# pdpatel13/Gravity-Simulator-using-MPI-Spark-and-CUDA

Measured on AMD Instinct MI355X. Metric: body-updates/sec (whole node) at N=1M direct O(N^2), 1/2/4/8 MI355X, higher is better.
Workload: dtype fp32

## Files before the change

### csrc/hip/nbody_sym.hip

```cpp
#include <hip/hip_runtime.h>
#include <stdint.h>
#include <stdlib.h>

#include "gravsim.h"
#include "gs_common.h"
#include "gs_kernels.h"
#include "gs_sym_tile.h"

namespace gs {
namespace {

template <typename T>
struct Shape;
template <>
struct Shape<float> {
  static constexpr int I = 8, W = kSymC / (64 * I), J = 2;
};
template <>
struct Shape<double> {
  static constexpr int W = 4, I = 8, J = 1;
};

template <typename T>
struct Geo {
  static constexpr int W = Shape<T>::W, I = Shape<T>::I, J = Shape<T>::J;
  static constexpr int kTileI = 64 * I;
  static constexpr int kTileJ = 64 * J;
  static constexpr int kThreads = 64 * W;
  static constexpr int kTilesPerChunk = kSymC / kTileJ;
  static constexpr int kTilesPerQuantum = 128 / kTileJ;
  static_assert(W * kTileI == kSymC, "one workgroup holds one chunk on its i side");
  static_assert(kTileJ <= 128 && 128 % kTileJ == 0, "a j-tile must not straddle quanta");
};

__device__ __forceinline__ int shell_len(int A, int NC) {
  const bool takes = (A < NC / 2) == ((A & 1) == 0);
  return takes ? NC / 2 : NC / 2 - 1;
}

template <typename T>
struct TileSeq {
  int A, NC, real_chunks, u, u1;
  bool diag;
  static constexpr int kT = Geo<T>::kTilesPerChunk;
  __device__ __forceinline__ int d() const { return diag ? 0 : 1 + u / kT; }
  __device__ __forceinline__ int t() const { return u % kT; }
  __device__ __forceinline__ int valid(int uu) const {
    if (!diag)
      while (uu < u1 && (A + 1 + uu / kT) % NC >= real_chunks) uu = (uu / kT + 1) * kT;
    return uu;
  }
  __device__ __forceinline__ bool done() const { return u >= u1; }
  __device__ __forceinline__ int64_t row0() const {
    const int B = diag ? A : (A + d()) % NC;
    return (int64_t)B * kSymC + t() * Geo<T>::kTileJ;
  }
  __device__ __forceinline__ void next() { u = valid(u + 1); }
};

template <typename V>
__device__ __forceinline__ void stage_store(V* dst, int b, const V& q) {
  const int j = b / 64, l = b % 64;
  dst[j * sym::kStagedRows + sym::staged_entry(l, 0)] = q;
  dst[j * sym::kStagedRows + sym::staged_entry(l, 1)] = q;
}

template <typename T>
constexpr bool kJpack = sizeof(T) == 4;

template <typename T>
using ISetK = typename std::conditional<kJpack<T>, sym::ISetP<Geo<T>::I>,
                                        sym::ISetT<T, Geo<T>::I>>::type;

template <typename T>
struct StageQ {
  static constexpr int kN = kJpack<T> ? 2 : 1;
  static constexpr int kThreads = kJpack<T> ? 64 : Geo<T>::kTileJ;
  sym::Vec4<T> q[kN];
  __device__ __forceinline__ void load(const sym::Vec4<T>* X4, int64_t row0, int t) {
#pragma unroll
    for (int k = 0; k < kN; ++k) q[k] = X4[row0 + k * 64 + t];
  }
  __device__ __forceinline__ void store(sym::Vec4<T>* dst, int t) const {
    if constexpr (kJpack<T>) {
      const float4 p0 = {q[0].x, q[1].x, q[0].y, q[1].y}, p1 = {q[0].z, q[1].z, q[0].w, q[1].w};
#pragma unroll
      for (int c = 0; c < 2; ++c) {
        const int e = sym::staged_entry(t, c);
        dst[2 * e] = p0;
        dst[2 * e + 1] = p1;
      }
    } else {
      stage_store(dst, t, q[0]);
    }
  }
};

template <typename T>
struct Smem {
  T slot[2][Geo<T>::W][3][Geo<T>::kTileJ];
  sym::Vec4<T> jt[2][Geo<T>::J * sym::kStagedRows];
};

template <typename T, bool SYM, bool EXACT>
__device__ __forceinline__ void run_tiles(const SymArgs& a, ISetK<T>& is, TileSeq<T> seq,
                                          int br, Smem<T>& sm) {
  using G = Geo<T>;
  using V4 = sym::Vec4<T>;
  constexpr int J = G::J;
  const int w = threadIdx.x >> 6, lane = threadIdx.x & 63;
  const V4* X4 = static_cast<const V4*>(a.X);
  const T eps2 = (T)a.eps2, cut2 = (T)a.cut2;
  int buf = 0, cur = 0;
  const bool stager = threadIdx.x < StageQ<T>::kThreads;
  if (!seq.done() && stager) {
    StageQ<T> sq;
    sq.load(X4, seq.row0(), threadIdx.x);
    sq.store(sm.jt[0], threadIdx.x);
  }
  __syncthreads();
  while (!seq.done()) {
    TileSeq<T> nx = seq;
    nx.next();
    const int d = seq.d(), t = seq.t();
    StageQ<T> q_next;
    const bool stage_next = !nx.done() && stager;
    if (stage_next) q_next.load(X4, nx.row0(), threadIdx.x);
    T cx[J], cy[J], cz[J];
    sym::CSetT<T, J> cs;
#pragma unroll
    for (int j = 0; j < J; ++j) cs.cx[j] = cs.cy[j] = cs.cz[j] = T(0);
    if constexpr (kJpack<T>) {
      sym::tile_lds_jp<G::I, SYM, EXACT>(is, cs, sm.jt[cur], eps2, sym::f2{a.cut_k, a.cut_c});
    } else {
      sym::tile_lds64<G::I, SYM, EXACT>(is, cs, sm.jt[cur], eps2, cut2);
    }
#pragma unroll
    for (int j = 0; j < J; ++j) { cx[j] = cs.cx[j]; cy[j] = cs.cy[j]; cz[j] = cs.cz[j]; }
    if constexpr (SYM) {
#pragma unroll
      for (int j = 0; j < J; ++j) {
        sm.slot[buf][w][0][j * 64 + lane] = cx[j];
        sm.slot[buf][w][1][j * 64 + lane] = cy[j];
        sm.slot[buf][w][2][j * 64 + lane] = cz[j];
      }
    }
    if (stage_next) q_next.store(sm.jt[cur ^ 1], threadIdx.x);
    __syncthreads();
    if constexpr (SYM) {
      T* pj = static_cast<T*>(a.Pj) + ((int64_t)br * a.H + (d - 1)) * 3 * kSymC;
      for (int v = threadIdx.x; v < 3 * G::kTileJ; v += G::kThreads) {
        const int c = v / G::kTileJ, b = v % G::kTileJ;
        T acc = sm.slot[buf][0][c][b];
#pragma unroll
        for (int u = 1; u < G::W; ++u) acc += sm.slot[buf][u][c][b];
        pj[(int64_t)c * kSymC + t * G::kTileJ + b] = acc;
      }
      buf ^= 1;
    }
    cur ^= 1;
    seq = nx;
  }
}

__device__ __forceinline__ bool local_first_unit(const SymArgs& a, int b, int* br, int* s,
                                                 int* stage, int* part) {
  const uint32_t m = (uint32_t)a.lf[b];
  const bool ring = a.gate_n > 1, halves = a.Kr > 0 && !ring;
  *br = (int)((m >> kUnitRowShift) & (uint32_t)kUnitRowMax);
  *s = (int)(m & (uint32_t)kUnitMax);
  *stage = ring ? (int)((m >> 28) & 7u) : 0;
  *part = halves && ((m >> 30) & 1u) ? (int)((m >> 28) & 3u) : -1;
  return (m >> 31) != 0u;
}

__device__ __forceinline__ bool gate_open_or_defer(const SymArgs& a, int b, int stage) {
  __shared__ int open_s;
  if (threadIdx.x == 0) {
    const bool open =
        __hip_atomic_load(a.gate + stage, __ATOMIC_ACQUIRE, __HIP_MEMORY_SCOPE_SYSTEM) != 0u;
    if (!open) {
      const unsigned k =
          __hip_atomic_fetch_add(a.defer, 1u, __ATOMIC_RELAXED, __HIP_MEMORY_SCOPE_AGENT);
      a.defer[1 + k] = (unsigned)b;
    }
    open_s = open ? 1 : 0;
  }
  __syncthreads();
  return open_s != 0;
}

__device__ __forceinline__ void audit_unit(const SymArgs& a, unsigned long long n = 1) {
  if (threadIdx.x == 0)
    __hip_atomic_fetch_add(a.audit, n, __ATOMIC_RELAXED, __HIP_MEMORY_SCOPE_AGENT);
}

template <typename T, bool EXACT>
__device__ __forceinline__ unsigned force_sym_body(const SymArgs& a, int b) {
  using G = Geo<T>;
  using V4 = sym::Vec4<T>;
  __shared__ Smem<T> sm;
  const int w = threadIdx.x >> 6, lane = threadIdx.x & 63;
  int br, s, stage = 0, part = -1;
  bool gated = false;
  if (a.units == 6) {
    gated = local_first_unit(a, b, &br, &s, &stage, &part) && a.gate != nullptr;
  } else if (a.units == 7) {
    local_first_unit(a, (int)a.defer[1 + a.defer_index], &br, &s, &stage, &part);
  } else {
    const int ns = a.S - a.Kr, shell = a.band_rows * ns, dg = a.band_rows * a.D;
    if (b < shell) {
      br = b / ns;
      s = b % ns;
    } else if (b < shell + dg) {
      const int k = b - shell;
      br = k / a.D;
      s = a.S + k % a.D;
    } else {
      const int k = b - shell - dg;
      part = k % a.Np;
      br = (k / a.Np) / a.Kr;
      s = ns + (k / a.Np) % a.Kr;
    }
  }
  const int A = a.a0 + a.band0 + br;
  const bool diag = s >= a.S;
  const bool split = !diag && s >= a.S - a.Kr;
  const unsigned long long weight = split && part < 0 ? (unsigned long long)a.Np : 1ull;
  const bool count_empty = a.audit != nullptr;
  if ((int64_t)A * kSymC >= a.n_real)
    return count_empty ? (unsigned)weight : 0u;
  const int seg_tiles = a.L * G::kTilesPerQuantum;
  TileSeq<T> seq{A, a.NC, a.real_chunks, 0, 0, diag};
  int u_lo = 0;
  if (diag) {
    const int q = s - a.S, plen = G::kTilesPerChunk / a.D;
    seq.u = q * plen;
    seq.u1 = seq.u + plen;
  } else {
    const int h_tiles = shell_len(A, a.NC) * G::kTilesPerChunk;
    const int u0 = s * seg_tiles;
    if (u0 >= h_tiles)
      return count_empty ? (unsigned)weight : 0u;
    seq.u1 = min(u0 + seg_tiles, h_tiles);
    u_lo = u0;
    seq.u = seq.valid(u0);
  }
  if (gated && !gate_open_or_defer(a, b, stage)) return 0u;
  const unsigned long long t_start = a.utrace ? __builtin_amdgcn_s_memrealtime() : 0ull;
  const V4* X4 = static_cast<const V4*>(a.X);
  ISetK<T> is;
  const int64_t i_row0 = (int64_t)A * kSymC + w * G::kTileI;
#pragma unroll
  for (int i = 0; i < G::I; ++i) {
    const V4 q = X4[i_row0 + i * 64 + lane];
    is.x[i] = q.x; is.y[i] = q.y; is.z[i] = q.z; is.mu[i] = q.w;
    is.ax[i] = is.ay[i] = is.az[i] = std::remove_reference_t<decltype(is.ax[i])>(0);
  }
  auto store_i = [&](T* out) {
#pragma unroll
    for (int i = 0; i < G::I; ++i) {
      const int b = w * G::kTileI + i * 64 + lane;
      if constexpr (kJpack<T>) {
        out[b] = is.ax[i].x + is.ax[i].y;
        out[kSymC + b] = is.ay[i].x + is.ay[i].y;
        out[2 * kSymC + b] = is.az[i].x + is.az[i].y;
      } else {
        out[b] = is.ax[i];
        out[kSymC + b] = is.ay[i];
        out[2 * kSymC + b] = is.az[i];
      }
    }
  };
  if (diag) {
    run_tiles<T, false, EXACT>(a, is, seq, br, sm);
    store_i(static_cast<T*>(a.Pd) + ((int64_t)br * a.D + (s - a.S)) * 3 * kSymC);
  } else {
    T* const pi = static_cast<T*>(a.Pi) + ((int64_t)br * a.S + s) * 3 * kSymC;
    T* const px = split ? static_cast<T*>(a.Px) +
                              ((int64_t)br * a.Kr + (s - (a.S - a.Kr))) * (a.Np - 1) * 3 * kSymC
                        : nullptr;
    const int pc0 = split && part > 0 ? part : 0;
    const int pc1 = !split ? 1 : part >= 0 ? part + 1 : a.Np;
    const int u_end = seq.u1;
#pragma unroll 1
    for (int pc = pc0; pc < pc1; ++pc) {
      TileSeq<T> sq = seq;
      if (split) {
        sq.u1 = min(u_lo + (pc + 1) * seg_tiles / a.Np, u_end);
        sq.u = sq.valid(min(u_lo + pc * seg_tiles / a.Np, u_end));
      }
      if (pc > pc0) {
#pragma unroll
        for (int i = 0; i < G::I; ++i)
          is.ax[i] = is.ay[i] = is.az[i] = std::remove_reference_t<decltype(is.ax[i])>(0);
      }
      run_tiles<T, true, EXACT>(a, is, sq, br, sm);
      store_i(pc == 0 ? pi : px + (int64_t)(pc - 1) * 3 * kSymC);
      if (pc + 1 < pc1) __syncthreads();

    }
  }
  if (a.utrace && threadIdx.x == 0) {
    const unsigned hw = __builtin_amdgcn_s_getreg((31 << 11) | 4);
    const unsigned xcc = __builtin_amdgcn_s_getreg((3 << 11) | 20);
    const int64_t slot = a.units == 7 ? (int64_t)a.trace_defer0 + a.defer_index : b;
    unsigned long long* e = a.utrace + 4 * slot;
    e[0] = t_start;
    e[1] = __builtin_amdgcn_s_memrealtime();
    e[2] = (unsigned long long)hw | ((unsigned long long)xcc << 32);
    e[3] = ((unsigned long long)(unsigned)br << 32) | (unsigned)s;
  }
  return a.audit ? (unsigned)weight : 0u;
}

struct ClockSpan {
  __device__ __forceinline__ static unsigned long long* slot() {
    __shared__ unsigned long long t0[3];
    return t0;
  }
  __device__ __forceinline__ static void begin(const SymArgs& a) {
    if (threadIdx.x == 0) {
      slot()[2] = reinterpret_cast<unsigned long long>(a.clk);
      if (a.clk) {
        slot()[0] = __builtin_amdgcn_s_memtime();
        slot()[1] = __builtin_amdgcn_s_memrealtime();
      }
    }
  }
  __device__ __forceinline__ static void end() {
    if (threadIdx.x == 0) {
      unsigned long long* clk = reinterpret_cast<unsigned long long*>(slot()[2]);
      if (clk) {
        const unsigned long long mt1 = __builtin_amdgcn_s_memtime();
        const unsigned long long rt1 = __builtin_amdgcn_s_memrealtime();
        __hip_atomic_fetch_add(clk, mt1 - slot()[0], __ATOMIC_RELAXED, __HIP_MEMORY_SCOPE_AGENT);
        __hip_atomic_fetch_add(clk + 1, rt1 - slot()[1], __ATOMIC_RELAXED,
                               __HIP_MEMORY_SCOPE_AGENT);
        __hip_atomic_fetch_add(clk + 2, 1ull, __ATOMIC_RELAXED, __HIP_MEMORY_SCOPE_AGENT);
      }
    }
  }
};

template <typename T, bool EXACT, bool DEFER, bool DYN, bool PF>
__device__ __forceinline__ void force_sym_entry(SymArgs a) {
  ClockSpan::begin(a);
  if constexpr (!DEFER && !DYN) {
    const unsigned w = force_sym_body<T, EXACT>(a, blockIdx.x);
    if (w) audit_unit(a, w);
  } else if constexpr (DYN && !PF) {
    __shared__ unsigned next_s;
    const int cap = (int)blockIdx.x < a.first_wave ? 1 : a.unit_cap;
    unsigned done = 0;
    for (int k = 0; k < cap; ++k) {
      if (threadIdx.x == 0)
        next_s = __hip_atomic_fetch_add(a.work, 1u, __ATOMIC_RELAXED, __HIP_MEMORY_SCOPE_AGENT);
      __syncthreads();
      const unsigned u = next_s;
      if (u >= (unsigned)a.n_units) break;
      done += force_sym_body<T, EXACT>(a, (int)u);
      __syncthreads();
    }
    if (done) audit_unit(a, done);
  } else if constexpr (DYN) {
    __shared__ unsigned next_s;
    const bool fw = (int)blockIdx.x < a.first_wave;
    const unsigned base = (unsigned)a.first_wave;
    auto fetch = [&]() -> unsigned {
      return base + __hip_atomic_fetch_add(a.work, 1u, __ATOMIC_RELAXED, __HIP_MEMORY_SCOPE_AGENT);
    };
    unsigned done = 0;
    if (fw && !a.persist) {
      if ((int)blockIdx.x < a.n_units) done += force_sym_body<T, EXACT>(a, (int)blockIdx.x);
    } else {
      if (!fw && threadIdx.x == 0) next_s = fetch();
      __syncthreads();
      unsigned u = fw ? (unsigned)blockIdx.x : next_s;
      const int cap = fw ? 0x7fffffff : a.unit_cap;
      for (int k = 0; k < cap && u < (unsigned)a.n_units; ++k) {
        const bool more = k + 1 < cap;
        const bool early = more && u + base < (unsigned)a.n_units;
        unsigned nx = ~0u;
        if (threadIdx.x == 0 && early) nx = fetch();
        done += force_sym_body<T, EXACT>(a, (int)u);
        __syncthreads();
        if (threadIdx.x == 0) next_s = early ? nx : more ? fetch() : ~0u;
        __syncthreads();
        u = next_s;
      }
    }
    if (done) audit_unit(a, done);
  } else {
    const unsigned n = a.defer[0];
    if (blockIdx.x == 0 && threadIdx.x == 0 && n > 0)
      __hip_atomic_fetch_max(a.defer_max, n, __ATOMIC_RELAXED, __HIP_MEMORY_SCOPE_AGENT);
    unsigned done = 0;
    for (unsigned k = blockIdx.x; k < n; k += gridDim.x) {
      a.defer_index = (int32_t)k;
      done += force_sym_body<T, EXACT>(a, 0);
      __syncthreads();
    }
    if (done) audit_unit(a, done);
  }
  ClockSpan::end();
}

template <bool EXACT, bool DEFER = false, bool DYN = false, bool PF = false>
__global__ __launch_bounds__(Geo<float>::kThreads) void force_sym_kernel_f32(SymArgs a) {
  force_sym_entry<float, EXACT, DEFER, DYN, PF>(a);
}
template <bool EXACT, bool DEFER = false, bool DYN = false, bool PF = false>
__global__ __launch_bounds__(Geo<double>::kThreads)
void force_sym_kernel_f64(SymArgs a) {
  force_sym_entry<double, EXACT, DEFER, DYN, PF>(a);
}


template <typename T, int C>
struct TreeAcc {
  static constexpr int kDepth = 9;
  T st[kDepth][C];
  unsigned pos;
  __device__ __forceinline__ void push(int level, T* v) {
    unsigned p = pos >> level;
#pragma unroll
    for (int k = 0; k < kDepth; ++k) {
      if (!(p & 1u)) break;
#pragma unroll
      for (int c = 0; c < C; ++c) v[c] = st[0][c] + v[c];
#pragma unroll
      for (int s = 0; s + 1 < kDepth; ++s)
#pragma unroll
        for (int c = 0; c < C; ++c) st[s][c] = st[s + 1][c];
      p >>= 1;
    }
#pragma unroll
    for (int s = kDepth - 1; s > 0; --s)
#pragma unroll
      for (int c = 0; c < C; ++c) st[s][c] = st[s - 1][c];
#pragma unroll
    for (int c = 0; c < C; ++c) st[0][c] = v[c];
    pos += 1u << level;
  }
  __device__ __forceinline__ void result(T* v) const {
#pragma unroll
    for (int c = 0; c < C; ++c) v[c] = st[0][c];
  }
};

template <typename T, int C, typename Leaf>
__device__ __forceinline__ void push_leaves(TreeAcc<T, C>& t, int lo, int n, Leaf&& leaf) {
  if (n >= 4) {
    for (int b = lo; b < lo + n; b += 4) {
      T v[4][C];
#pragma unroll
      for (int j = 0; j < 4; ++j) leaf(b + j, v[j]);
#pragma unroll
      for (int c = 0; c < C; ++c) v[0][c] = (v[0][c] + v[1][c]) + (v[2][c] + v[3][c]);
      t.push(2, v[0]);
    }
  } else {
    for (int b = lo; b < lo + n; ++b) {
      T v[C];
      leaf(b, v);
      t.push(0, v);
    }
  }
}

template <typename A, typename T>
__device__ __forceinline__ A ld(const T* p) {
  return *reinterpret_cast<const A*>(p);
}

template <bool NT, typename A, typename T>
__device__ __forceinline__ A ld_pj(const T* p) {
  if constexpr (NT && std::is_same<A, T>::value) return __builtin_nontemporal_load(p);
  else return *reinterpret_cast<const A*>(p);
}

template <typename T, int C, typename A = T, bool NT = false>
__device__ __forceinline__ void pj_range_add(const SymArgs& a, int A_lo, int A_hi, int X,
                                             int wrap, const T* pjc, int64_t comp_stride,
                                             A* out) {
  constexpr int U = 8;
  const int64_t step = (int64_t)(a.H - 1) * 3 * kSymC;
  const T* p0 = pjc + ((int64_t)(A_lo - a.a0 - a.band0) * a.H + (X - A_lo + wrap - 1)) * 3 * kSymC;
  for (int A0 = A_lo; A0 < A_hi; A0 += U, p0 += U * step) {
    A v[U][C];
#pragma unroll
    for (int u = 0; u < U; ++u) {
      const int Ar = A0 + u;
      const int d = X - Ar + wrap;
      const bool ok = Ar < A_hi && (d != a.NC / 2 || shell_len(Ar, a.NC) == a.NC / 2);
      const T* p = p0 + u * step;
#pragma unroll
      for (int k = 0; k < C; ++k) v[u][k] = ok ? ld_pj<NT, A>(p + k * comp_stride) : A(0);
    }
#pragma unroll
    for (int u = 0; u < U; ++u)
#pragma unroll
      for (int k = 0; k < C; ++k) out[k] += v[u][k];
  }
}

template <typename T, int C, typename A = T, bool NT = false>
__device__ __forceinline__ void pj_row_sum(const SymArgs& a, int A_lo, int A_hi, int X,
                                           const T* pjc, int64_t comp_stride, A* out) {
#pragma unroll
  for (int k = 0; k < C; ++k) out[k] = A(0);
  const int s0 = X - a.NC / 2;
  if (s0 >= 0) {
    pj_range_add<T, C, A, NT>(a, max(A_lo, s0), min(A_hi, X), X, 0, pjc, comp_stride, out);
  } else {
    pj_range_add<T, C, A, NT>(a, A_lo, min(A_hi, X), X, 0, pjc, comp_stride, out);
    pj_range_add<T, C, A, NT>(a, max(A_lo, s0 + a.NC), A_hi, X, a.NC, pjc, comp_stride, out);
  }
}

__device__ __forceinline__ int sym_row_owner(const SymArgs& a, int X) {
  const int blk = X / a.RB;
  int q = 0;
  while (q + 1 < a.P && a.blk_lo[q + 1] <= blk) ++q;
  return q;
}

template <typename T>
__global__ __launch_bounds__(256) void sym_block_reduce_kernel(SymArgs a) {
  const int64_t nb = (int64_t)a.real_chunks * kSymC;
  const int64_t x = (int64_t)blockIdx.x * 256 + threadIdx.x;
  if (x >= nb) return;
  const int X = (int)(x / kSymC), c = (int)(x % kSymC);
  const int b = (a.a0 + a.band0) / a.RB + (int)blockIdx.y;
  const int A_lo = max(b * a.RB, 0), A_hi = min((b + 1) * a.RB, a.real_chunks);
  T v[3];
  pj_row_sum<T, 3>(a, A_lo, max(A_lo, A_hi), X, static_cast<const T*>(a.Pj) + c, kSymC, v);
  T* o = static_cast<T*>(a.Bbuf) + (int64_t)(b - a.blk_lo[a.rank]) * 3 * nb + x;
  o[0] = v[0];
  o[nb] = v[1];
  o[2 * nb] = v[2];
}

template <typename T, bool NT>
__device__ __forceinline__ void sym_node_reduce_body(const SymArgs& a, int bx, int by) {
  if (a.sig && bx == 0 && by == 0 && threadIdx.x == 0) {
    __builtin_amdgcn_fence(__ATOMIC_RELEASE, "");
    asm volatile("s_waitcnt vmcnt(0)" ::: "memory");
    __hip_atomic_fetch_add(a.sig, 1u, __ATOMIC_RELAXED, __HIP_MEMORY_SCOPE_SYSTEM);
  }
  const int64_t nb = (int64_t)a.real_chunks * kSymC;
  const int64_t tx = (int64_t)bx * 256 + threadIdx.x;
  if (a.x_count > 0 && tx >= a.x_count) return;
  int64_t x = a.x_lo + tx;
  if (x >= (int64_t)a.NC * kSymC) x -= (int64_t)a.NC * kSymC;
  if (x >= nb) return;
  const int X = (int)(x / kSymC), c = (int)(x % kSymC);
  const int own_lo = a.blk_lo[a.rank], own_hi = a.blk_lo[a.rank + 1];
  int lo = own_lo, l = sym_dyadic_level(lo, own_hi);
  for (int k = 0; k < by; ++k) {
    lo += 1 << l;
    l = sym_dyadic_level(lo, own_hi);
  }
  TreeAcc<T, 3> t;
  t.pos = 0;
  const T* Bb = static_cast<const T*>(a.Bbuf);
  const T* pjc = static_cast<const T*>(a.Pj) + c;
  auto leaf = [&](int b, T* v) {
    if (Bb) {
      const T* p = Bb + (int64_t)(b - own_lo) * 3 * nb + x;
      v[0] = p[0];
      v[1] = p[nb];
      v[2] = p[2 * nb];
    } else {
      const int A_lo = b * a.RB, A_hi = min((b + 1) * a.RB, a.real_chunks);
      pj_row_sum<T, 3, T, NT>(a, A_lo, max(A_lo, A_hi), X, pjc, kSymC, v);
    }
  };
  push_leaves(t, lo, 1 << l, leaf);
  T r[3];
  t.result(r);
  const int q = sym_row_owner(a, X);
  const int64_t bq = (int64_t)a.blk_lo[q] * a.RB * kSymC;
  const int64_t nlq = (int64_t)(a.blk_lo[q + 1] - a.blk_lo[q]) * a.RB * kSymC;
  T* o = static_cast<T*>(a.Sbuf) + (int64_t)a.nn * 3 * bq + (int64_t)by * 3 * nlq + (x - bq);
  o[0] = r[0];
  o[nlq] = r[1];
  o[2 * nlq] = r[2];
}

template <typename T, bool NT>
__global__ __launch_bounds__(256) void sym_node_reduce_kernel(SymArgs a) {
  sym_node_reduce_body<T, NT>(a, (int)blockIdx.x, (int)blockIdx.y);
}

template <typename T>
__device__ __forceinline__ void sym_tree_all(const SymArgs& a, int64_t li, T* S) {
  TreeAcc<T, 3> t;
  t.pos = 0;
  const T* R = static_cast<const T*>(a.Rbuf) + li;
  const T* own = static_cast<const T*>(a.Sbuf) + (int64_t)a.nn * 3 * a.i_begin + li;
  int j = 0;
  for (int q = 0; q < a.P; ++q) {
    const int hi = a.blk_lo[q + 1];
    const int j0 = j;
    for (int lo = a.blk_lo[q]; lo < hi; ++j) {
      const int l = sym_dyadic_level(lo, hi);
      const T* p = q == a.rank ? own + (int64_t)(j - j0) * 3 * a.n_local
                               : R + (int64_t)j * 3 * a.n_local;
      T v[3] = {p[0], p[a.n_local], p[2 * a.n_local]};
      t.push(l, v);
      lo += 1 << l;
    }
  }
  t.result(S);
}

template <typename T, typename A = T>
__device__ __forceinline__ A split_parts_add(const SymArgs& a, int br, int s, int segs,
                                             int64_t off, const T* p, A acc) {
  const T* px =
      static_cast<const T*>(a.Px) + (int64_t)br * a.Kr * (a.Np - 1) * 3 * kSymC + off;
  for (; s < segs; ++s) {
    const int sp = s - (a.S - a.Kr);
    A t = ld<A>(p + (int64_t)s * 3 * kSymC);
    for (int q = 0; q + 1 < a.Np; ++q) t += ld<A>(px + ((int64_t)sp * (a.Np - 1) + q) * 3 * kSymC);
    acc += t;
  }
  return acc;
}

__device__ __forceinline__ int ti_mid(const SymArgs& a, int segs, int ns) {
  if (a.NC > 32) return ns;
  const int loads = a.D + ns + (segs - ns) * a.Np + a.NC / 2;
  const int m = loads / 2 - a.D;
  return m < 0 ? 0 : (m > ns ? ns : m);
}

template <typename T>
__device__ __forceinline__ T pi_range_add(const T* __restrict__ p, int s0, int s1, T acc) {
  constexpr int U = 8;
  int s = s0;
  for (; s + U <= s1; s += U) {
    T v[U];
#pragma unroll
    for (int u = 0; u < U; ++u) v[u] = __builtin_nontemporal_load(p + (int64_t)(s + u) * 3 * kSymC);
#pragma unroll
    for (int u = 0; u < U; ++u) acc += v[u];
  }
  for (; s < s1; ++s) acc += __builtin_nontemporal_load(p + (int64_t)s * 3 * kSymC);
  return acc;
}

template <typename T>
__device__ __forceinline__ T ti_half0(const SymArgs& a, int br, int k, int c, int m) {
  const T* __restrict__ pd = static_cast<const T*>(a.Pd) + (int64_t)br * a.D * 3 * kSymC +
                             k * kSymC + c;
  T acc = pd[0];
  for (int q = 1; q < a.D; ++q) acc += pd[q * 3 * kSymC];
  const T* p = static_cast<const T*>(a.Pi) + (int64_t)br * a.S * 3 * kSymC + k * kSymC + c;
  return pi_range_add(p, 0, m, acc);
}
template <typename T>
__device__ __forceinline__ T ti_half1(const SymArgs& a, int br, int k, int c, int m, int ns,
                                      int segs) {
  const T* p = static_cast<const T*>(a.Pi) + (int64_t)br * a.S * 3 * kSymC + k * kSymC + c;
  T acc = pi_range_add(p, m, ns, T(0));
  if (ns < segs) acc = split_parts_add(a, br, ns, segs, k * kSymC + c, p, acc);
  return acc;
}

template <typename T>
__device__ __forceinline__ void sym_row_reduce_body(const SymArgs& a, int bx, int k) {
  const int64_t b = (int64_t)bx * 256 + threadIdx.x;
  if (b >= (int64_t)a.band_rows * kSymC) return;
  const int br = (int)(b / kSymC), c = (int)(b % kSymC);
  const int A = a.a0 + a.band0 + br;
  if ((int64_t)A * kSymC >= a.n_real) return;
  const int segs = (16 * shell_len(A, a.NC) + a.L - 1) / a.L;
  const int ns = min(segs, a.S - a.Kr);
  const int m = ti_mid(a, segs, ns);
  const T h0 = ti_half0<T>(a, br, k, c, m);
  const T h1 = ti_half1<T>(a, br, k, c, m, ns, segs);
  static_cast<T*>(a.Ti)[(int64_t)k * a.n_local + (int64_t)(a.band0 + br) * kSymC + c] = h0 + h1;
}

template <typename T>
__global__ __launch_bounds__(256) void sym_row_reduce_kernel(SymArgs a) {
  sym_row_reduce_body<T>(a, (int)blockIdx.x, (int)blockIdx.y);
}

template <typename T, bool NT>
__global__ __launch_bounds__(256) void sym_node_row_kernel(SymArgs a, int node_bx, int row_bx) {
  const int nnb = node_bx * a.nn;
  if ((int)blockIdx.x < nnb) {
    sym_node_reduce_body<T, NT>(a, (int)blockIdx.x % node_bx, (int)blockIdx.x / node_bx);
  } else {
    const int k = (int)blockIdx.x - nnb;
    sym_row_reduce_body<T>(a, k % row_bx, k / row_bx);
  }
}

template <typename T>
__global__ __launch_bounds__(256) void sym_finalize_kernel(SymArgs a) {
  using V4 = sym::Vec4<T>;
  const int64_t li = (int64_t)blockIdx.x * 256 + threadIdx.x;
  if (a.gate && li < a.gate_n)
    __hip_atomic_store(a.gate + li, 0u, __ATOMIC_RELAXED, __HIP_MEMORY_SCOPE_AGENT);
  if (a.gate && li == 0) __hip_atomic_store(a.defer, 0u, __ATOMIC_RELAXED, __HIP_MEMORY_SCOPE_AGENT);
  if (a.work && li == 0) __hip_atomic_store(a.work, 0u, __ATOMIC_RELAXED, __HIP_MEMORY_SCOPE_AGENT);
  if (li >= a.n_local) return;
  const int64_t gi = a.i_begin + li;
  V4* vel = static_cast<V4*>(a.vel);
  const V4 zero = {T(0), T(0), T(0), T(0)};
  if (gi >= a.n_real) {
    if (a.acc_out) {
      static_cast<V4*>(a.acc_out)[li] = zero;
    } else {
      vel[li] = zero;
      static_cast<V4*>(a.X_next)[gi] = zero;
    }
    return;
  }
  const T* ti = static_cast<const T*>(a.Ti) + li;
  T S[3];
  sym_tree_all<T>(a, li, S);
  const T ax = ti[0] + S[0], ay = ti[a.n_local] + S[1], az = ti[2 * a.n_local] + S[2];
  if (a.acc_out) {
    static_cast<V4*>(a.acc_out)[li] = V4{ax, ay, az, T(0)};
    return;
  }
  const T dt = (T)a.dt;
  const V4 xi = static_cast<const V4*>(a.X)[gi];
  V4 v = vel[li];
  v.x = v.x + ax * dt;
  v.y = v.y + ay * dt;
  v.z = v.z + az * dt;
  V4 xn;
  xn.x = xi.x + v.x * dt;
  xn.y = xi.y + v.y * dt;
  xn.z = xi.z + v.z * dt;
  xn.w = xi.w;
  vel[li] = v;
  static_cast<V4*>(a.X_next)[gi] = xn;
}

template <typename T, bool SPLIT>
__global__ __launch_bounds__(SPLIT ? 384 : 192) void sym_tail_kernel(SymArgs a) {
  using V4 = sym::Vec4<T>;
  __shared__ T h1_s[3][64], s_s[3][64], acc_s[3][64];
  const int w = threadIdx.x >> 6, l = threadIdx.x & 63;
  const int k = w % 3, half = w / 3;
  const int64_t li = (int64_t)blockIdx.x * 64 + l;
  if (a.gate && blockIdx.x == 0 && (int)threadIdx.x < a.gate_n)
    __hip_atomic_store(a.gate + threadIdx.x, 0u, __ATOMIC_RELAXED, __HIP_MEMORY_SCOPE_AGENT);
  if (a.gate && blockIdx.x == 0 && threadIdx.x == 0)
    __hip_atomic_store(a.defer, 0u, __ATOMIC_RELAXED, __HIP_MEMORY_SCOPE_AGENT);
  if (a.work && blockIdx.x == 0 && threadIdx.x == 0)
    __hip_atomic_store(a.work, 0u, __ATOMIC_RELAXED, __HIP_MEMORY_SCOPE_AGENT);
  const int64_t gi = a.i_begin + li;
  const bool real = li < a.n_local && gi < a.n_real;
  T h = T(0);
  if (real) {
    const int X = (int)(gi / kSymC), c = (int)(gi % kSymC);
    const int br = X - a.a0;
    const int segs = (16 * shell_len(X, a.NC) + a.L - 1) / a.L;
    const int ns = min(segs, a.S - a.Kr);
    const int m = ti_mid(a, segs, ns);
    if (half == 0) h = ti_half0<T>(a, br, k, c, m);
    if (half == 1 || !SPLIT) {
      h1_s[k][l] = ti_half1<T>(a, br, k, c, m, ns, segs);
      TreeAcc<T, 1> t;
      t.pos = 0;
      const T* pjc = static_cast<const T*>(a.Pj) + k * kSymC + c;
      push_leaves(t, 0, a.B, [&](int b, T* v) {
        const int A_lo = b * a.RB, A_hi = min((b + 1) * a.RB, a.real_chunks);
        pj_row_sum<T, 1>(a, A_lo, max(A_lo, A_hi), X, pjc, kSymC, v);
      });
      T S[1];
      t.result(S);
      s_s[k][l] = S[0];
    }
  }
  __syncthreads();
  if (real && half == 0) acc_s[k][l] = (h + h1_s[k][l]) + s_s[k][l];
  __syncthreads();
  if (w != 0 || li >= a.n_local) return;
  V4* vel = static_cast<V4*>(a.vel);
  const V4 zero = {T(0), T(0), T(0), T(0)};
  if (!real) {
    if (a.acc_out) {
      static_cast<V4*>(a.acc_out)[li] = zero;
    } else {
      vel[li] = zero;
      static_cast<V4*>(a.X_next)[gi] = zero;
    }
    return;
  }
  const T ax = acc_s[0][l], ay = acc_s[1][l], az = acc_s[2][l];
  if (a.acc_out) {
    static_cast<V4*>(a.acc_out)[li] = V4{ax, ay, az, T(0)};
    return;
  }
  const T dt = (T)a.dt;
  const V4 xi = static_cast<const V4*>(a.X)[gi];
  V4 v = vel[li];
  v.x = v.x + ax * dt;
  v.y = v.y + ay * dt;
  v.z = v.z + az * dt;
  V4 xn;
  xn.x = xi.x + v.x * dt;
  xn.y = xi.y + v.y * dt;
  xn.z = xi.z + v.z * dt;
  xn.w = xi.w;
  vel[li] = v;
  static_cast<V4*>(a.X_next)[gi] = xn;
}

template <typename T>
hipError_t launch_force_sym_t(const SymArgs& a, hipStream_t s) {
  int units = a.band_rows * (a.S + a.D);
  if (a.Kr > 0 && (a.units == 0 || (a.units == 6 && a.gate_n <= 1)))
    units += a.band_rows * a.Kr * (a.Np - 1);
  if (a.units >= 6 && (a.band_rows != a.rows || !a.lf)) return hipErrorInvalidValue;
  if (a.units == 7) units = a.defer_grid;
  if (units <= 0) return hipSuccess;
  SymArgs b = a;
  b.n_units = units;
  unsigned g = (unsigned)units;
  if (a.work && (a.units == 0 || a.units == 6) && a.unit_cap > 1 && units > a.first_wave) {
    if (!a.work_zero) {
      const hipError_t e = hipMemsetAsync(a.work, 0, sizeof(unsigned), s);
      if (e != hipSuccess) return e;
    }
    const int64_t rest = units - a.first_wave;
    const int64_t more = (5 * rest + 4LL * a.unit_cap - 1) / (4LL * a.unit_cap);
    g = (unsigned)(a.first_wave + (more < rest ? more : rest));
    b.persist = a.persist && (int64_t)units > 128LL * a.first_wave ? 1 : 0;
    if (b.persist) g = (unsigned)a.first_wave;
  } else {
    b.work = nullptr;
    b.persist = 0;
  }
  const dim3 grid(g), block(Geo<T>::kThreads);
  const bool d = a.units == 7, y = b.work != nullptr;
  const bool pf = y && (b.persist || (int64_t)units <= 128LL * (a.first_wave > 0 ? a.first_wave : 1));
  if constexpr (sizeof(T) == 8) {
    if (a.exact) {
      if (d) hipLaunchKernelGGL((force_sym_kernel_f64<true, true>), grid, block, 0, s, b);
      else if (pf) hipLaunchKernelGGL((force_sym_kernel_f64<true, false, true, true>), grid, block, 0, s, b);
      else if (y) hipLaunchKernelGGL((force_sym_kernel_f64<true, false, true>), grid, block, 0, s, b);
      else hipLaunchKernelGGL((force_sym_kernel_f64<true>), grid, block, 0, s, b);
    } else {
      if (d) hipLaunchKernelGGL((force_sym_kernel_f64<false, true>), grid, block, 0, s, b);
      else if (pf) hipLaunchKernelGGL((force_sym_kernel_f64<false, false, true, true>), grid, block, 0, s, b);
      else if (y) hipLaunchKernelGGL((force_sym_kernel_f64<false, false, true>), grid, block, 0, s, b);
      else hipLaunchKernelGGL((force_sym_kernel_f64<false>), grid, block, 0, s, b);
    }
  } else {
    if (a.exact) {
      if (d) hipLaunchKernelGGL((force_sym_kernel_f32<true, true>), grid, block, 0, s, b);
      else if (pf) hipLaunchKernelGGL((force_sym_kernel_f32<true, false, true, true>), grid, block, 0, s, b);
      else if (y) hipLaunchKernelGGL((force_sym_kernel_f32<true, false, true>), grid, block, 0, s, b);
      else hipLaunchKernelGGL((force_sym_kernel_f32<true>), grid, block, 0, s, b);
    } else {
      if (d) hipLaunchKernelGGL((force_sym_kernel_f32<false, true>), grid, block, 0, s, b);
      else if (pf) hipLaunchKernelGGL((force_sym_kernel_f32<false, false, true, true>), grid, block, 0, s, b);
      else if (y) hipLaunchKernelGGL((force_sym_kernel_f32<false, false, true>), grid, block, 0, s, b);
      else hipLaunchKernelGGL((force_sym_kernel_f32<false>), grid, block, 0, s, b);
    }
  }
  return hipGetLastError();
}

}

hipError_t launch_force_sym(const SymArgs& a, hipStream_t s) {
  return a.fp64 ? launch_force_sym_t<double>(a, s) : launch_force_sym_t<float>(a, s);
}

}

extern "C" int gs_sym_tile_shape(int32_t fp64, int32_t* waves, int32_t* ipl, int32_t* jpl) {
  using namespace gs;
  if (waves) *waves = fp64 ? Geo<double>::W : Geo<float>::W;
  if (ipl) *ipl = fp64 ? Geo<double>::I : Geo<float>::I;
  if (jpl) *jpl = fp64 ? Geo<double>::J : Geo<float>::J;
  return 0;
}

namespace gs {

hipError_t launch_sym_block_reduce(const SymArgs& a, hipStream_t s) {
  if (!a.Bbuf || a.band_rows % a.RB || (a.a0 + a.band0) % a.RB) return hipErrorInvalidValue;
  const int64_t bodies = (int64_t)a.real_chunks * kSymC;
  const dim3 grid((unsigned)((bodies + 255) / 256), (unsigned)(a.band_rows / a.RB));
  if (a.fp64) hipLaunchKernelGGL(sym_block_reduce_kernel<double>, grid, dim3(256), 0, s, a);
  else hipLaunchKernelGGL(sym_block_reduce_kernel<float>, grid, dim3(256), 0, s, a);
  return hipGetLastError();
}

hipError_t launch_sym_node_reduce(const SymArgs& a, hipStream_t s) {
  if (!a.Bbuf && (a.band0 != 0 || a.band_rows != a.rows)) return hipErrorInvalidValue;
  const int64_t nb = (int64_t)a.real_chunks * kSymC;
  const int64_t bodies = a.x_count > 0 ? a.x_count : nb;
  if (bodies <= 0) return hipSuccess;
  const dim3 grid((unsigned)((bodies + 255) / 256), (unsigned)a.nn);
  const bool nt = a.P > 2;
  if (a.fp64) {
    if (nt) hipLaunchKernelGGL((sym_node_reduce_kernel<double, true>), grid, dim3(256), 0, s, a);
    else hipLaunchKernelGGL((sym_node_reduce_kernel<double, false>), grid, dim3(256), 0, s, a);
  } else {
    if (nt) hipLaunchKernelGGL((sym_node_reduce_kernel<float, true>), grid, dim3(256), 0, s, a);
    else hipLaunchKernelGGL((sym_node_reduce_kernel<float, false>), grid, dim3(256), 0, s, a);
  }
  return hipGetLastError();
}

hipError_t launch_sym_node_row(const SymArgs& a, hipStream_t s) {
  if (!a.Bbuf && (a.band0 != 0 || a.band_rows != a.rows)) return hipErrorInvalidValue;
  const int64_t nb = (int64_t)a.real_chunks * kSymC;
  const int64_t bodies = a.x_count > 0 ? a.x_count : nb;
  const int node_bx = (int)((bodies + 255) / 256);
  const int row_bx = (int)(((int64_t)a.band_rows * kSymC + 255) / 256);
  const dim3 grid((unsigned)(node_bx * a.nn + 3 * row_bx));
  const bool nt = a.P > 2;
  if (a.fp64) {
    if (nt) hipLaunchKernelGGL((sym_node_row_kernel<double, true>), grid, dim3(256), 0, s, a, node_bx, row_bx);
    else hipLaunchKernelGGL((sym_node_row_kernel<double, false>), grid, dim3(256), 0, s, a, node_bx, row_bx);
  } else {
    if (nt) hipLaunchKernelGGL((sym_node_row_kernel<float, true>), grid, dim3(256), 0, s, a, node_bx, row_bx);
    else hipLaunchKernelGGL((sym_node_row_kernel<float, false>), grid, dim3(256), 0, s, a, node_bx, row_bx);
  }
  return hipGetLastError();
}

hipError_t launch_sym_row_reduce(const SymArgs& a, hipStream_t s) {
  const int64_t bodies = (int64_t)a.band_rows * kSymC;
  const dim3 grid((unsigned)((bodies + 255) / 256), 3);
  if (a.fp64) hipLaunchKernelGGL(sym_row_reduce_kernel<double>, grid, dim3(256), 0, s, a);
  else hipLaunchKernelGGL(sym_row_reduce_kernel<float>, grid, dim3(256), 0, s, a);
  return hipGetLastError();
}

hipError_t launch_sym_finalize(const SymArgs& a, hipStream_t s) {
  const dim3 grid((unsigned)((a.n_local + 255) / 256));
  if (a.fp64) hipLaunchKernelGGL(sym_finalize_kernel<double>, grid, dim3(256), 0, s, a);
  else hipLaunchKernelGGL(sym_finalize_kernel<float>, grid, dim3(256), 0, s, a);
  return hipGetLastError();
}

hipError_t launch_sym_tail(const SymArgs& a, hipStream_t s, bool split) {
  if (a.P != 1 || a.band_rows != a.rows) return hipErrorInvalidValue;
  const dim3 grid((unsigned)((a.n_local + 63) / 64));
  if (split) {
    if (a.fp64) hipLaunchKernelGGL((sym_tail_kernel<double, true>), grid, dim3(384), 0, s, a);
    else hipLaunchKernelGGL((sym_tail_kernel<float, true>), grid, dim3(384), 0, s, a);
  } else {
    if (a.fp64) hipLaunchKernelGGL((sym_tail_kernel<double, false>), grid, dim3(192), 0, s, a);
    else hipLaunchKernelGGL((sym_tail_kernel<float, false>), grid, dim3(192), 0, s, a);
  }
  return hipGetLastError();
}

int sym_occupancy(int fp64) {
  int n = 0;
  const hipError_t e =
      fp64 ? hipOccupancyMaxActiveBlocksPerMultiprocessor(&n, force_sym_kernel_f64<false>,
                                                          Geo<double>::kThreads, 0)
           : hipOccupancyMaxActiveBlocksPerMultiprocessor(&n, force_sym_kernel_f32<false>,
                                                          Geo<float>::kThreads, 0);
  return e == hipSuccess ? n : 0;
}

}
```

Before: 6.447 million.

## Process two j-tiles per barrier round in symmetric tile loop

Measured after the change: 6.444 million. About the same (-0.1%).

```diff
diff --git a/csrc/hip/nbody_sym.hip b/csrc/hip/nbody_sym.hip
--- a/csrc/hip/nbody_sym.hip
+++ b/csrc/hip/nbody_sym.hip
@@ -41,7 +41,7 @@
 template <typename T>
 struct TileSeq {
   int A, NC, real_chunks, u, u1;
-  bool diag;
+  int diag;
   static constexpr int kT = Geo<T>::kTilesPerChunk;
   __device__ __forceinline__ int d() const { return diag ? 0 : 1 + u / kT; }
   __device__ __forceinline__ int t() const { return u % kT; }
@@ -96,10 +96,12 @@
   }
 };
 
+constexpr int kRound = 2;
+
 template <typename T>
 struct Smem {
-  T slot[2][Geo<T>::W][3][Geo<T>::kTileJ];
-  sym::Vec4<T> jt[2][Geo<T>::J * sym::kStagedRows];
+  T slot[2][Geo<T>::W][3][kRound * Geo<T>::kTileJ];
+  sym::Vec4<T> jt[2][kRound * Geo<T>::J * sym::kStagedRows];
 };
 
 template <typename T, bool SYM, bool EXACT>
@@ -108,58 +110,79 @@
   using G = Geo<T>;
   using V4 = sym::Vec4<T>;
   constexpr int J = G::J;
+  constexpr int kTileRows = J * sym::kStagedRows;
   const int w = threadIdx.x >> 6, lane = threadIdx.x & 63;
   const V4* X4 = static_cast<const V4*>(a.X);
   const T eps2 = (T)a.eps2, cut2 = (T)a.cut2;
   int buf = 0, cur = 0;
   const bool stager = threadIdx.x < StageQ<T>::kThreads;
-  if (!seq.done() && stager) {
+  TileSeq<T> sa = seq, sb = seq;
+  if (!sb.done()) sb.next();
+  if (stager) {
     StageQ<T> sq;
-    sq.load(X4, seq.row0(), threadIdx.x);
-    sq.store(sm.jt[0], threadIdx.x);
+    if (!sa.done()) {
+      sq.load(X4, sa.row0(), threadIdx.x);
+      sq.store(sm.jt[0], threadIdx.x);
+    }
+    if (!sb.done()) {
+      sq.load(X4, sb.row0(), threadIdx.x);
+      sq.store(sm.jt[0] + kTileRows, threadIdx.x);
+    }
   }
   __syncthreads();
-  while (!seq.done()) {
-    TileSeq<T> nx = seq;
-    nx.next();
-    const int d = seq.d(), t = seq.t();
-    StageQ<T> q_next;
-    const bool stage_next = !nx.done() && stager;
-    if (stage_next) q_next.load(X4, nx.row0(), threadIdx.x);
-    T cx[J], cy[J], cz[J];
-    sym::CSetT<T, J> cs;
-#pragma unroll
-    for (int j = 0; j < J; ++j) cs.cx[j] = cs.cy[j] = cs.cz[j] = T(0);
-    if constexpr (kJpack<T>) {
-      sym::tile_lds_jp<G::I, SYM, EXACT>(is, cs, sm.jt[cur], eps2, sym::f2{a.cut_k, a.cut_c});
-    } else {
-      sym::tile_lds64<G::I, SYM, EXACT>(is, cs, sm.jt[cur], eps2, cut2);
-    }
-#pragma unroll
-    for (int j = 0; j < J; ++j) { cx[j] = cs.cx[j]; cy[j] = cs.cy[j]; cz[j] = cs.cz[j]; }
-    if constexpr (SYM) {
-#pragma unroll
-      for (int j = 0; j < J; ++j) {
-        sm.slot[buf][w][0][j * 64 + lane] = cx[j];
-        sm.slot[buf][w][1][j * 64 + lane] = cy[j];
-        sm.slot[buf][w][2][j * 64 + lane] = cz[j];
+  while (!sa.done()) {
+    const int n = sb.done() ? 1 : 2;
+    TileSeq<T> na = sb, nb = sb;
+    if (!na.done()) na.next();
+    nb = na;
+    if (!nb.done()) nb.next();
+#pragma unroll 1
+    for (int h = 0; h < n; ++h) {
+      StageQ<T> q_next;
+      const TileSeq<T> st = h ? nb : na;
+      const bool stage_next = !st.done() && stager;
+      if (stage_next) q_next.load(X4, st.row0(), threadIdx.x);
+      T cx[J], cy[J], cz[J];
+      sym::CSetT<T, J> cs;
+#pragma unroll
+      for (int j = 0; j < J; ++j) cs.cx[j] = cs.cy[j] = cs.cz[j] = T(0);
+      const V4* tile = sm.jt[cur] + h * kTileRows;
+      if constexpr (kJpack<T>) {
+        sym::tile_lds_jp<G::I, SYM, EXACT>(is, cs, tile, eps2, sym::f2{a.cut_k, a.cut_c});
+      } else {
+        sym::tile_lds64<G::I, SYM, EXACT>(is, cs, tile, eps2, cut2);
       }
-    }
-    if (stage_next) q_next.store(sm.jt[cur ^ 1], threadIdx.x);
+#pragma unroll
+      for (int j = 0; j < J; ++j) { cx[j] = cs.cx[j]; cy[j] = cs.cy[j]; cz[j] = cs.cz[j]; }
+      if constexpr (SYM) {
+#pragma unroll
+        for (int j = 0; j < J; ++j) {
+          sm.slot[buf][w][0][h * G::kTileJ + j * 64 + lane] = cx[j];
+          sm.slot[buf][w][1][h * G::kTileJ + j * 64 + lane] = cy[j];
+          sm.slot[buf][w][2][h * G::kTileJ + j * 64 + lane] = cz[j];
+        }
+      }
+      if (stage_next) q_next.store(sm.jt[cur ^ 1] + h * kTileRows, threadIdx.x);
+    }
     __syncthreads();
     if constexpr (SYM) {
-      T* pj = static_cast<T*>(a.Pj) + ((int64_t)br * a.H + (d - 1)) * 3 * kSymC;
-      for (int v = threadIdx.x; v < 3 * G::kTileJ; v += G::kThreads) {
-        const int c = v / G::kTileJ, b = v % G::kTileJ;
-        T acc = sm.slot[buf][0][c][b];
-#pragma unroll
-        for (int u = 1; u < G::W; ++u) acc += sm.slot[buf][u][c][b];
-        pj[(int64_t)c * kSymC + t * G::kTileJ + b] = acc;
+      constexpr int kT = G::kTilesPerChunk;
+      T* pj = static_cast<T*>(a.Pj) + (int64_t)br * a.H * 3 * kSymC;
+      const int ua = sa.u, ub = sb.u;
+      for (int v = threadIdx.x; v < n * 3 * G::kTileJ; v += G::kThreads) {
+        const int h = v / (3 * G::kTileJ), r = v % (3 * G::kTileJ);
+        const int c = r / G::kTileJ, b = r % G::kTileJ;
+        const int u = h ? ub : ua;
+        T acc = sm.slot[buf][0][c][h * G::kTileJ + b];
+#pragma unroll
+        for (int k = 1; k < G::W; ++k) acc += sm.slot[buf][k][c][h * G::kTileJ + b];
+        pj[((int64_t)(u / kT) * 3 + c) * kSymC + (u % kT) * G::kTileJ + b] = acc;
       }
       buf ^= 1;
     }
     cur ^= 1;
-    seq = nx;
+    sa = na;
+    sb = nb;
   }
 }
 
```
